# VKoskiv/c-ray

Measured on AMD Instinct MI355X. Metric: Mray/s (primary+secondary), higher is better.
Workload: dtype f32; 1 GPU; input/hdr.json 1280x720, 256 spp, 8 bounces (BASELINE.json configs[1]); venusscaled.obj = generated 524288-triangle stand-in (tools/gen_assets.py), HDR env map + 2048^2 grid texture from the reference tree; environment map: a generated stand-in of the HDR's size (tools/cfg2_blob.py — no reference tree to flatten hdr.json from): the same paths and rays, other radiance; parallelism=1 rank: the whole frame in one dispatch

## Files before the change

### c-ray_amd/csrc/cray_hip.hip

```cpp
#include <hip/hip_runtime.h>
#include <dlfcn.h>

#include <algorithm>
#include <chrono>
#include <cmath>
#include <cstdio>
#include <cstring>
#include <condition_variable>
#include <atomic>
#include <cassert>
#include <memory>
#include <mutex>
#include <thread>
#include <string>
#include <vector>

#include "cray_hip.h"
#define CRH_EM_POW_TABLES_IN_LDS
#include "pt_device.h"
#include "scene_compile.h"
#include "ctx_access.h"

using namespace crh;

// ... 929 lines not shown
	UP(prog, cs.prog.data(), cs.prog.size());
	UP(textures, cs.textures.data(), cs.textures.size());
	{
		void *texDev = nullptr;
		rc = takeTexels ? takeTexels(&texDev) : CRH_OK;
		if (rc) { freeScene(c); return rc; }
		if (texDev) { c->sceneAllocs.push_back(texDev); d.texels = (const f4 *)texDev; }
		else UP(texels, cs.texels.data(), cs.texels.size());
	}
#undef UP
	d.tlas_first = cs.tlas_first;
	d.material_count = (uint32_t)cs.materials.size(); d.bsdf_count = (uint32_t)cs.bsdfs.size(); d.const_count = (uint32_t)cs.consts.size();
	d.image_count = (uint32_t)cs.images.size(); d.texture_count = (uint32_t)cs.textures.size();
	d.tlas_root = cs.tlas_root; d.tlas_node_count = cs.tlas_node_count; d.tlas_prim_base = cs.tlas_prim_base; d.shade_classes = cs.shade_classes; d.instance_count = (uint32_t)cs.instances.size();
	d.background = cs.background;
	{ const crh_camera *cam = nullptr; rc = upload(c, &cs.camera, 1, &cam); if (rc) { freeScene(c); return rc; } d.camera = cam; }
	c->d = d;
	c->haveWide = !cs.wide.empty(); c->wideTlasRoot = cs.wide_tlas_root;
	if (cs.want_wide && !c->haveWide && !cs.wide_refused.empty())
		fprintf(stderr, "libcray_hip: CRH_WALK_WIDE4 was asked for, but this scene has no 4-ary copy (%s): the binary walk renders it\n", cs.wide_refused.c_str());
	c->hasPrograms = cs.prog.size() > 1 || cs.has_volumes || getenv("CRH_FORCE_PROGRAMS") != nullptr;
	c->hasVolumes = cs.has_volumes;
	c->aovDepth = cs.max_albedo_depth;
	c->haveScene = true;
	*tCopiesMs = upMs();
	rc = preloadKernel(c, true);
	if (rc != CRH_OK) return rc;
	unsigned int flag = 0;
	HIP_TRY(hipMemcpy(&flag, c->dWork + (CRH_WORK_SLOTS - 1), sizeof(flag), hipMemcpyDeviceToHost));
	return CRH_OK;
}
// ... 1428 lines not shown
```

### c-ray_amd/csrc/pathtrace_roll.h

```cpp
#pragma once

#define CRH_ROLL_HITS_MAX 136u
#define CRH_ROLL_IDS_MISSES (CRH_IDS_HITS + 2u * CRH_ROLL_HITS_MAX)
#define CRH_ROLL_IDS_BYTES (CRH_ROLL_IDS_MISSES + 128u)
#ifndef CRH_ROLL_SLOTS
#define CRH_ROLL_SLOTS 4u
#endif
#ifndef CRH_ROLL_FIFO
#define CRH_ROLL_FIFO 0
#endif
#define CRH_ROLL_SLOT_SHIFT 30u
#define CRH_ROLL_ITEM_MASK 0x3FFFFFFFu


template <int LEVEL, int WPS, bool PROG, int SAMP, bool WIDE = false>
__global__ __launch_bounds__(CRH_BLOCK, CRH_WPS_OVERRIDE) void k_pathtrace_roll(const DScene Sarg, const crh_render_params P, const BlockQueue Q, float *fb,
																 unsigned long long *counters,
																 float *stage, int chunk, unsigned long long *waveStats, const Sched K, float *queues, uint32_t *ovfAll, unsigned int *errFlag) {
	__shared__ uint32_t s_stack[CRH_STACK_LDS * CRH_BLOCK];
	__shared__ uint32_t s_park[CRH_PARK_SLOTS * CRH_BLOCK];
	enum { RQ_RAYS, RQ_HITS, RQ_MISSES, RQ_FREE, RQ_CLS_LO, RQ_CLS_HI,
	       RQ_GENLEFT,
	       RQ_FLAGS,
	       RQ_HEAD,
	       RQ_OPEN,
	       RQ_GEN,
	       RQ_DRY,
	       RQ_SLOT0 };
	enum { SJ_X0, SJ_Y0, SJ_WH , SJ_BWBH , SJ_PASS0, SJ_PASSN, SJ_NEXT, SJ_OUT,
	       SJ_BASE_LO, SJ_BASE_HI,
	       SJ_WORDS };
	enum { SJ_WH_DEFER = 1 << 30 };
	enum { SJ_WH_H_MASK = 0x3FFF };
#define CRH_RQ_IS_DRY(v) ((v) != 0)
	enum { NS = (int)CRH_ROLL_SLOTS, RQ_WORDS = RQ_SLOT0 + NS * SJ_WORDS };
	static_assert(NS >= 2 && NS <= 4, "2..4 job slots (two bits of the item word)");
	static_assert((CRH_STACK_LDS + CRH_PARK_SLOTS) * CRH_BLOCK * 4 + (CRH_BLOCK / 64) * (CRH_ROLL_IDS_BYTES + RQ_WORDS * 4) + 512 + 256 + CRH_INST_LDS_BYTES + CRH_SHADE_LDS_BYTES <= 40960, "4 blocks per CU share 160 KB of LDS (incl. powf's tables)");
	const DScene S = globalize(Sarg);
	CRH_EM_POW_TABLES_INIT();
	const unsigned long long tStart = wall_clock64();
	uint32_t unitsDone = 0;
#ifdef CRH_EXP_ABS_TIMES
	unsigned long long tDry = 0;
	bool snapDone = false;
#endif
	LdsStack stk;
	stk.lds = (lds_u32 *)&s_stack[threadIdx.x];
	stk.parkp = (lds_u32 *)&s_park[threadIdx.x];
	CRH_STAGE_SHADE_TABLES();
	CRH_STAGE_INSTANCE_TABLES();
	CountersT<LEVEL, PROG, WIDE> cnt;
	memset(&cnt, 0, sizeof(cnt));
	const uint32_t lane = threadIdx.x & 63u;
	const uint32_t wave = (blockIdx.x * CRH_BLOCK + threadIdx.x) >> 6;
	__shared__ uint8_t s_cls[256];
	const bool sorted = K.sortFrom > 0 && S.shade_classes >= (uint32_t)K.sortFrom && S.instance_count <= 256u;
	if (sorted) {
		for (uint32_t i = threadIdx.x; i < S.instance_count; i += CRH_BLOCK) s_cls[i] = (uint8_t)CRH_DINST_CLASS(S.instances[i].kind);
		__syncthreads();
	}
	stk.ovf = (glb_u32 *)ovfAll + (size_t)__builtin_amdgcn_readfirstlane(wave) * CRH_OVF_WORDS_PER_WAVE;
	const size_t slabFloats = (size_t)Q.bw * Q.bh * chunk * 3;
	float *const myStage = stage + (size_t)__builtin_amdgcn_readfirstlane(wave) * (size_t)NS * slabFloats;
	const int passEnd = P.first_pass + P.pass_count;
	const uint32_t trisOff = (uint32_t)((const char *)S.tris - (const char *)S.nodes);
	constexpr bool LEANTAB = CRH_PATH_LEAN && !PROG;
// ... 36 lines not shown
		if (open > 0) {
			lds_int *gj = wq + RQ_SLOT0 + wq[RQ_GEN] * SJ_WORDS, *oj = wq + RQ_SLOT0 + head * SJ_WORDS;
			const int gb = gj[SJ_BWBH], ob = oj[SJ_BWBH];
			left = (gb & 0xFFFF) * (gb >> 16) * gj[SJ_PASSN] - gj[SJ_NEXT];
			if (left < 0) left = 0;
			moreChunks = !(gj[SJ_WH] & SJ_WH_DEFER) && gj[SJ_PASS0] + gj[SJ_PASSN] < passEnd;
			if (oj[SJ_NEXT] >= (ob & 0xFFFF) * (ob >> 16) * oj[SJ_PASSN] && oj[SJ_OUT] == 0 && (open > 1 || !moreChunks)) flags |= 1;
		}
		if (open < NS && (!CRH_RQ_IS_DRY(wq[RQ_DRY]) || moreChunks)) flags |= 2;
		wq[RQ_GENLEFT] = left; wq[RQ_FLAGS] = flags;
	};

	if (lane == 0) {
		wq[RQ_RAYS] = 0; wq[RQ_HITS] = 0; wq[RQ_MISSES] = 0; wq[RQ_FREE] = (int)CRH_PATHS; wq[RQ_CLS_LO] = 0; wq[RQ_CLS_HI] = 0;
		wq[RQ_HEAD] = 0; wq[RQ_OPEN] = 0; wq[RQ_GEN] = 0; wq[RQ_DRY] = 0;
		for (int i = 0; i < NS * SJ_WORDS; ++i) wq[RQ_SLOT0 + i] = 0;
		refreshJobWords();
	}
	for (uint32_t i = lane; i < CRH_PATHS; i += 64u) ids[i] = (uint8_t)i;
	__threadfence_block();
	Walk w;
	memset(&w, 0, sizeof(w));
	w.phase = PH_IDLE;
	uint32_t myPath = 0;
	auto retireRefill = [&](int &rq, int &hq, int &mq) __attribute__((always_inline)) {
		const bool fin = (w.phase == PH_SHADE);
		const bool finHit = fin && w.hit.inst >= 0, finMiss = fin && w.hit.inst < 0;
		const unsigned long long hm = __ballot(finHit), mm = __ballot(finMiss);
		uint32_t cls = 0;
		if (fin) {
// ... 34 lines not shown
		if (idle && (int)er < take) {
			myPath = myRay;
#else
		if (idle && (int)er < take) {
			myPath = ids[CRH_IDS_RAYS + (uint32_t)(rq - take) + er];
#endif
			const f4 *q = tab.rec(myPath);
			const f4 q0 = q[0], q1 = q[1];
			{ TablePort<SAMP> port2{tab.rec(myPath)}; walkBegin(S, w, stk, v3{q0.x, q0.y, q0.z}, v3{q1.x, q1.y, q1.z}, cnt, port2, (uint32_t)K.rayFlags); }
			if constexpr (LEVEL >= 2) {
				if (dumpRays && dumpCount + er < dumpCap) { float *o = dumpRays + (size_t)(dumpCount + er) * 6u; o[0] = q0.x; o[1] = q0.y; o[2] = q0.z; o[3] = q1.x; o[4] = q1.y; o[5] = q1.z; }
			}
		}
		if constexpr (LEVEL >= 2) dumpCount += (uint32_t)take;
		hq += (int)__popcll(hm); mq += (int)__popcll(mm); rq -= take;
		if (lane == 0) { wq[RQ_HITS] = hq; wq[RQ_MISSES] = mq; wq[RQ_RAYS] = rq; }
		__threadfence_block();
	};
	uint32_t guard = (uint32_t)K.roundLimit;
	for (;;) {
		if (--guard == 0u) { if (lane == 0) atomicOr(errFlag, CRH_ERRFLAG_ROUND_LIMIT); break; }
#ifdef CRH_EXP_ABS_TIMES
		if (waveStats && !snapDone && (guard & 15u) == 0u) {
			uint32_t handedOut = 0;
			if (lane == 0) handedOut = __hip_atomic_load((uint32_t *)Q.counter, __ATOMIC_RELAXED, __HIP_MEMORY_SCOPE_AGENT);
			handedOut = __builtin_amdgcn_readfirstlane(handedOut);
			if (handedOut >= Q.total) {
				snapDone = true;
				if (lane == 0) {
					const int head = wq[RQ_HEAD], open = wq[RQ_OPEN];
					unsigned long long notGenerated = 0, notStaged = 0;
// ... 59 lines not shown
					const bool isT = nTw >= K.triInRun && w.phase == PH_TRI;
					if constexpr (LEVEL >= 2) {
						if (lane == 0) { CRH_WCTR(11, 1); CRH_WCTR(17, now); }
#ifdef CRH_CENSUS
						const uint32_t wf = (uint32_t)__popcll(__ballot(w.phase == PH_SHADE || w.phase == PH_IDLE));
						if (lane == 0) { CRH_WCTR(30, nTw >= K.triInRun ? 0u : (uint32_t)nTw); CRH_WCTR(31, wf); if (nTw >= K.triInRun) { CRH_WCTR(26, 1); CRH_WCTR(27, nTw); } }
#endif
					}
					if (isN || isT) {
						const uint32_t off = isN ? (uint32_t)(w.node << (WIDE ? 4 : 5)) : trisOff + w.pA * 48u;
						const char *rec = (const char *)S.nodes + off;
						q0 = *(const f4 *)rec; q1 = *(const f4 *)(rec + 16); q2 = *(const f4 *)(rec + 32); q3 = *(const f4 *)(rec + 48);
						if (WIDE || isT) { q4 = *(const f4 *)(rec + 64); q5 = *(const f4 *)(rec + 80); }
						if (WIDE && isN) { q6 = *(const f4 *)(rec + 96); q7 = *(const f4 *)(rec + 112); }
					}
					if constexpr (WIDE) { if (isN) stepWideLoaded<true>(S, w, stk, cnt, port, q0, q1, q2, q3, q4, q5, q6, q7); }
					else
					if (isN) stepNodeLoaded<true>(S, w, stk, cnt, port, q0, q1, q2, q3);
					if (isT) stepTriLoaded(S, w, stk, cnt, port, q0, q1, q2, q3, q4, q5);
					if ((int)__popcll(__ballot(w.phase == PH_CTRL)) >= K.ctrlInRun) {
#ifdef CRH_CENSUS
						if constexpr (LEVEL >= 2) { const uint32_t n2 = (uint32_t)__popcll(__ballot(w.phase == PH_CTRL)); if (lane == 0) { CRH_WCTR(28, 1); CRH_WCTR(29, n2); } }
#endif
						if (w.phase == PH_CTRL) stepCtrl(S, w, stk, cnt, port);
					}
					{
						const int nFi = (int)__popcll(__ballot(w.phase == PH_SHADE)), nEi = (int)__popcll(__ballot(w.phase == PH_IDLE));
						if (nFi + nEi >= K.swapInRun && (nFi > 0 || rqRun > 0) && hqRun < 64 && mqRun < 64) {
							if constexpr (LEVEL >= 2) { if (lane == 0) { CRH_WCTR(21, 1); CRH_WCTR(23, nFi + min(nEi + nFi, rqRun)); } }
							retireRefill(rqRun, hqRun, mqRun);
							port = TablePort<SAMP>{tab.rec(myPath)};
						}
					}
					now = __popcll(__ballot(w.phase == PH_NODE));
// ... 87 lines not shown
				const BlockJob J = loadJob(g);
				const uint32_t genNext = (uint32_t)wq[RQ_SLOT0 + g * SJ_WORDS + SJ_NEXT], genItems = genNext + (uint32_t)itemsLeft;
				const uint32_t item = genNext + lane;
				int x = 0, y = 0, pass = 0;
				const bool valid = item < genItems && decodeItem(J, item, x, y, pass);
				const unsigned long long vm = __ballot(valid);
				const int n = (int)__popcll(vm);
				if constexpr (COOP_STORE) {
					f4 q0 = f4{0.0f, 0.0f, 0.0f, 0.0f}, q1 = q0, q2 = q0, q3 = q0;
					uint32_t id = 0;
					if (valid) {
						const uint32_t rk = laneRank(vm);
						id = ids[CRH_IDS_FREE_END - (uint32_t)freeQ + rk];
						v3 ro, rd;
						PathRecT<RngT<SAMP>> r;
						beginPath(S, P, x, y, pass, ro, rd, r, cnt);
						packPathRay(q0, q1, q2, q3, ro, rd, r, item | ((uint32_t)g << CRH_ROLL_SLOT_SHIFT));
						ids[CRH_IDS_RAYS + (uint32_t)raysQ + rk] = (uint8_t)id;
					}
					tab.storeRec4(id, valid, q0, q1, q2, q3);
				} else
				if (valid) {
					const uint32_t rk = laneRank(vm);
					const uint32_t id = ids[CRH_IDS_FREE_END - (uint32_t)freeQ + rk];
					v3 ro, rd;
					PathRecT<RngT<SAMP>> r;
					beginPath(S, P, x, y, pass, ro, rd, r, cnt);
					putPathRay(tab.rec(id), ro, rd, r, item | ((uint32_t)g << CRH_ROLL_SLOT_SHIFT));
					ids[CRH_IDS_RAYS + (uint32_t)raysQ + rk] = (uint8_t)id;
				}
				if (lane == 0) {
					wq[RQ_RAYS] = raysQ + n; wq[RQ_FREE] = freeQ - n;
					lds_int *j = wq + RQ_SLOT0 + g * SJ_WORDS;
					j[SJ_NEXT] = (int)(genNext + 64u); j[SJ_OUT] = j[SJ_OUT] + n;
					refreshJobWords();
				}
				__threadfence_block();
				break;
			}
			case ST_MISS: {
				const int n = min(missQn, 64);
				int mySlot = -1;
				const bool have = (int)lane < n;
				uint32_t id = 0;
				f4 q0, q1, q2, q3;
				if constexpr (COOP_LOAD_MISS) {
					if (have) id = ids[CRH_ROLL_IDS_MISSES + (uint32_t)(missQn - n) + lane];
					tab.loadRec4(id, have, q0, q1, q2, q3);
				}
// ... 163 lines not shown
	}
	if (waveStats && lane == 0) {
#ifdef CRH_EXP_ABS_TIMES
		const unsigned long long tEnd = wall_clock64();
		waveStats[2 * wave] = tStart;
		waveStats[2 * wave + 1] = (((tDry ? tDry : tEnd) - tStart) << 32) | ((tEnd - tStart) & 0xFFFFFFFFull);
		if (!snapDone) { const size_t waves = (size_t)gridDim.x * (CRH_BLOCK / 64u); waveStats[2 * (waves + wave)] = 0; waveStats[2 * (waves + wave) + 1] = 0; }
#else
		waveStats[2 * wave] = wall_clock64() - tStart;
		waveStats[2 * wave + 1] = unitsDone;
#endif
	}
	const bool lead = (lane == 0);
	if constexpr (LEVEL >= 2) { if (dumpRays && lead) waveStats[CRH_DUMP_HDR + 2 + wave] = min(dumpCount, dumpCap); }
	uint32_t v;
	v = waveSum(cnt.paths); if (lead && v) atomicAdd(&counters[0], (unsigned long long)v);
	v = waveSum(cnt.rays); if (lead && v) atomicAdd(&counters[1], (unsigned long long)v);
	if constexpr (LEVEL >= 2) {
		v = waveSum(cnt.node_tests); if (lead && v) atomicAdd(&counters[2], (unsigned long long)v);
		v = waveSum(cnt.tri_tests); if (lead && v) atomicAdd(&counters[3], (unsigned long long)v);
		v = waveSum(cnt.inst_visits); if (lead && v) atomicAdd(&counters[4], (unsigned long long)v);
		v = waveSum(cnt.inst_hits); if (lead && v) atomicAdd(&counters[5], (unsigned long long)v);
		v = waveSum(cnt.sphere_tests); if (lead && v) atomicAdd(&counters[6], (unsigned long long)v);
		v = waveSum(cnt.tex_fetches); if (lead && v) atomicAdd(&counters[7], (unsigned long long)v);
	}
}
#undef CRH_WCTR
```

### c-ray_amd/csrc/pt_device.h

```cpp
#pragma once
#include <stdint.h>
#include <math.h>
#include <float.h>
#include <type_traits>
#include <utility>
#include "cray_hip.h"
#include "exact_math.h"

#if defined(__HIPCC__)
#define CRH_DEV __device__ __forceinline__
#define CRH_DEV_NOINLINE __device__ __noinline__
#define CRH_MEM __device__ __forceinline__
#else
#define CRH_MEM inline __attribute__((always_inline))
#define CRH_DEV static inline __attribute__((always_inline))
#define CRH_DEV_NOINLINE static __attribute__((noinline))
#endif

namespace crh {

#define CRH_PI 3.141592653589793238462643383279502f
#define CRH_NONE 0xFFFFFFFFu

struct alignas(16) f4 { float x, y, z, w; };
// ... 97 lines not shown
	uint32_t t_setup, t_trav, t_shade;
	uint32_t w_node, w_tri, w_ctrl, w_round, w_shade, w_setup;
	uint32_t u_node, u_shade;
	uint32_t t_swap, t_gen, n_swap, n_gen, u_swap, u_tri, u_ctrl;
#ifdef CRH_CENSUS
	uint32_t w_tri_in, u_tri_in, w_ctrl_in, u_ctrl_in;
	uint32_t u_wait_tri, u_wait_fin;
#endif
};
template <bool PROGRAMS, bool WIDE> struct CountersT<1, PROGRAMS, WIDE> {
	static constexpr int level = 1;
	static constexpr bool programs = PROGRAMS;
	static constexpr bool wide = WIDE;
	uint32_t rays, paths;
};
typedef CountersT<2, true> Counters;
typedef CountersT<1, true> LiteCounters;
struct NoCounters { static constexpr int level = 0; static constexpr bool programs = true; static constexpr bool wide = false; };
template <class T> struct cnt_traits { static constexpr int level = T::level; static constexpr bool programs = T::programs; static constexpr bool wide = T::wide; };
template <class T> struct cnt_traits<T &> { static constexpr int level = T::level; static constexpr bool programs = T::programs; static constexpr bool wide = T::wide; };
#define CRH_COUNT(c, field, n) do { if constexpr (crh::cnt_traits<decltype(c)>::level >= 2) (c).field += (n); } while (0)
#if defined(__HIPCC__)
#define CRH_TICK() ((uint32_t)wall_clock64())
#else
#define CRH_TICK() 0u
#endif
#define CRH_COUNT1(c, field, n) do { if constexpr (crh::cnt_traits<decltype(c)>::level >= 1) (c).field += (n); } while (0)

CRH_DEV v3 vadd(v3 a, v3 b) { return v3{a.x + b.x, a.y + b.y, a.z + b.z}; }
CRH_DEV v3 vsub(v3 a, v3 b) { return v3{a.x - b.x, a.y - b.y, a.z - b.z}; }
// ... 226 lines not shown
			  (m.c.x * v.x) + (m.c.y * v.y) + (m.c.z * v.z)};
}
CRH_DEV v3 xfVectorT(v3 v, const InstLine &m) {
	return v3{(m.a.x * v.x) + (m.b.x * v.y) + (m.c.x * v.z),
			  (m.a.y * v.x) + (m.b.y * v.y) + (m.c.y * v.z),
			  (m.a.z * v.x) + (m.b.z * v.y) + (m.c.z * v.z)};
}

CRH_DEV float triangleDistribution(float v) {
	const float orig = v * 2.0f - 1.0f;
	v = orig / sqrtf(fabsf(orig));
	v = rmin(rmax(v, -1.0f), 1.0f);
	v = v - ((orig >= 0.0f) ? 1.0f : -1.0f);
	return v;
}
template <class R>
CRH_DEV void getCameraRay(const crh_camera &cam, R &rng, int x, int y, v3 &ro, v3 &rd) {
	const v3 right = v3{cam.right[0], cam.right[1], cam.right[2]};
	const v3 up = v3{cam.up[0], cam.up[1], cam.up[2]};
	const v3 forward = v3{cam.forward[0], cam.forward[1], cam.forward[2]};
	v3 start = v3{0.0f, 0.0f, 0.0f};
	const float jitterX = triangleDistribution(getDimension(rng));
	const float jitterY = triangleDistribution(getDimension(rng));
	v3 pixX = vscale(right, (cam.sensor[0] / (float)cam.width));
	v3 pixY = vscale(up, (cam.sensor[1] / (float)cam.height));
	v3 pixV = vadd(forward, vadd(vscale(pixX, (float)x - (float)cam.width * 0.5f + jitterX + 0.5f),
								 vscale(pixY, (float)y - (float)cam.height * 0.5f + jitterY + 0.5f)));
	v3 dir = vnorm(pixV);
	if (cam.aperture > 0.0f) {
		float ft = cam.focal_distance / vdot(dir, forward);
		v3 focusPoint = alongRay(start, dir, ft);
		v2 disc = randomCoordOnUnitDisc(rng);
		v2 lensPoint = v2{disc.x * cam.aperture, disc.y * cam.aperture};
		start = vadd(start, vadd(vscale(right, lensPoint.x), vscale(up, lensPoint.y)));
		dir = vnorm(vsub(focusPoint, start));
	}
	ro = xfPoint(start, cam.A);
	rd = xfVector(dir, cam.A);
}

CRH_DEV uint32_t wrapIndex(int i, uint32_t W, uint32_t m64) {
	if ((W & (W - 1u)) == 0u) return (uint32_t)i & (W - 1u);
// ... 378 lines not shown
	RayK k;
	uint32_t node;
	uint32_t pA, pAe, pB, pBe;
	uint32_t sp, spBase;
	uint32_t inBlas, instFound;
	int32_t curInst;
	TravHit hit;
};

struct NullPort {
	CRH_MEM float draw() { return 0.5f; }
	CRH_MEM void save(int, uint32_t) {}
	CRH_MEM uint32_t load(int) { return 0u; }
};
enum { VP_T, VP_U, VP_V, VP_SLOT, VP_T1, VP_WORDS };
enum { BLAS_NONE = 0, BLAS_SOLID = 1, BLAS_VOL_ENTRY = 2, BLAS_VOL_EXIT = 3 };

template <class Cnt>
CRH_DEV bool sphereTest(const v3 o, const v3 d, float radius, float bound, float &t, Cnt &cnt) {
	CRH_COUNT(cnt, sphere_tests, 1);
	const float A = vdot(d, d);
	const float B = 2.0f * vdot(d, o);
	const float C = vdot(o, o) - (radius * radius);
	const float disc = B * B - 4.0f * A * C;
	if (disc < 0.0f) return false;
	const float sq = sqrtf(disc);
	float t0 = (-B + sq) / 2.0f;
	const float t1 = (-B - sq) / 2.0f;
	if (t0 > t1 && t1 > 0.0f) t0 = t1;
	if (t0 < 0.00001f || t0 > bound) return false;
	t = t0;
// ... 31 lines not shown
		return false;
	}
	if (w.inBlas == BLAS_VOL_EXIT && found) {
		float t1 = asF32(port.load(VP_T1));
		if (t1 < 0.0f) t1 = 0.0f;
		const float distanceInsideVolume = tWalk;
		const float hitDistance = -(1.0f / instDensity(instLine(S, stk, w.curInst, 1))) * em::logf_(port.draw());
		if (hitDistance < distanceInsideVolume) {
			w.hit.t = t1 + hitDistance; w.hit.u = 0.0f; w.hit.v = 0.0f; w.hit.slot = -2; w.hit.inst = w.curInst;
			CRH_COUNT(cnt, inst_hits, 1);
		}
	}
	return false;
}

template <class Stack, class Cnt, class Port>
CRH_DEV void walkAdvance(const DScene &S, Walk &w, Stack &stk, Cnt &cnt, Port &port) {
	if (w.pA != w.pAe) { w.phase = w.inBlas ? PH_TRI : PH_CTRL; return; }
	if constexpr (cnt_traits<Cnt>::wide) {
		if (w.node == CRH_NONE && w.sp > w.spBase) {
			const uint32_t e = stk.pop(--w.sp);
			if (e & CRH_WREF_LEAF) { w.pA = e & CRH_WREF_FIRST_MASK; w.pAe = w.pA + ((e >> CRH_WREF_COUNT_SHIFT) & CRH_WREF_COUNT_MAX); w.phase = w.inBlas ? PH_TRI : PH_CTRL; return; }
			w.node = e;
		}
	} else {
		if (w.node == CRH_NONE && w.sp > w.spBase) w.node = stk.pop(--w.sp);
	}
	if (w.node != CRH_NONE) { w.phase = w.k.oct >> CRH_RAY_PHASE_SHIFT; return; }
	if (!w.inBlas) { w.phase = PH_SHADE; return; }
	if constexpr (cnt_traits<Cnt>::programs) {
		if (__builtin_expect(w.inBlas >= BLAS_VOL_ENTRY, 0)) { if (volumeAdvance(S, w, stk, cnt, port)) return; }
	}
	if (w.instFound) { w.hit.inst = w.curInst; CRH_COUNT(cnt, inst_hits, 1); }
// ... 91 lines not shown
	walkAdvance(S, w, stk, cnt, port);
}
template <bool FAST = true, class Stack, class Cnt, class Port>
CRH_DEV void stepWide(const DScene &S, Walk &w, Stack &stk, Cnt &cnt, Port &port) {
	const char *rec = (const char *)S.nodes + (uint32_t)(w.node << 4);
	const f4 a0 = *(const f4 *)rec, a1 = *(const f4 *)(rec + 16), b0 = *(const f4 *)(rec + 32), b1 = *(const f4 *)(rec + 48);
	const f4 c0 = *(const f4 *)(rec + 64), c1 = *(const f4 *)(rec + 80), d0 = *(const f4 *)(rec + 96), d1 = *(const f4 *)(rec + 112);
	stepWideLoaded<FAST>(S, w, stk, cnt, port, a0, a1, b0, b1, c0, c1, d0, d1);
}
template <bool FAST, class Stack, class Cnt, class Port>
CRH_DEV void stepNodeAny(const DScene &S, Walk &w, Stack &stk, Cnt &cnt, Port &port) {
	if constexpr (cnt_traits<Cnt>::wide) stepWide<FAST>(S, w, stk, cnt, port); else stepNode<FAST>(S, w, stk, cnt, port);
}

template <class Cnt>
CRH_DEV void testTriangle(const f4 q0, const f4 q1, const f4 q2, uint32_t slot, Walk &w, Cnt &cnt) {
	const v3 v0 = v3{q0.x, q0.y, q0.z}, e1 = v3{q0.w, q1.x, q1.y}, e2 = v3{q1.z, q1.w, q2.x}, n = v3{q2.y, q2.z, q2.w};
	CRH_COUNT(cnt, tri_tests, 1);
	const v3 c = vsub(v0, w.k.o);
	const v3 r = vcross(w.k.d, c);
	const float invDet = 1.0f / vdot(n, w.k.d);
	const float u = vdot(r, e2) * invDet;
	const float v = vdot(r, e1) * invDet;
	if (u >= 0.0f && v >= 0.0f && u + v <= 1.0f) {
		const float t = vdot(n, c) * invDet;
		if (t >= 0.0f && t < w.hit.t) { w.hit.t = t; w.hit.u = u; w.hit.v = v; w.hit.slot = (int32_t)slot; w.instFound = 1; }
	}
}
template <class Stack, class Cnt, class Port>
CRH_DEV void stepTriLoaded(const DScene &S, Walk &w, Stack &stk, Cnt &cnt, Port &port, const f4 a0, const f4 a1, const f4 a2, const f4 b0, const f4 b1, const f4 b2) {
	const uint32_t slot = w.pA;
	const bool two = slot + 1u < w.pAe;
	const uint32_t slot2 = two ? slot + 1u : slot;
	w.pA = slot2 + 1u;
	if (w.pA == w.pAe) { w.pA = w.pB; w.pAe = w.pBe; w.pB = w.pBe = 0; }
	testTriangle(a0, a1, a2, slot, w, cnt);
	if (two) testTriangle(b0, b1, b2, slot2, w, cnt);
	walkAdvance(S, w, stk, cnt, port);
}
template <class Stack, class Cnt, class Port>
CRH_DEV void stepTri(const DScene &S, Walk &w, Stack &stk, Cnt &cnt, Port &port) {
	const uint32_t slot = w.pA;
	const uint32_t slot2 = slot + 1u < w.pAe ? slot + 1u : slot;
	const char *ta = (const char *)S.tris + (uint32_t)(slot * 48u), *tb = (const char *)S.tris + (uint32_t)(slot2 * 48u);
	const f4 a0 = *(const f4 *)ta, a1 = *(const f4 *)(ta + 16), a2 = *(const f4 *)(ta + 32);
	const f4 b0 = *(const f4 *)tb, b1 = *(const f4 *)(tb + 16), b2 = *(const f4 *)(tb + 32);
	stepTriLoaded(S, w, stk, cnt, port, a0, a1, a2, b0, b1, b2);
}

template <class Stack, class Cnt, class Port>
CRH_DEV void stepCtrl(const DScene &S, Walk &w, Stack &stk, Cnt &cnt, Port &port) {
	const uint32_t slot = w.pA++;
	if (w.pA == w.pAe) { w.pA = w.pB; w.pAe = w.pBe; w.pB = w.pBe = 0; }
	const int32_t idx = (int32_t)(slot - S.tlas_prim_base);
	const InstLine inst = instLine(S, stk, idx, 0);
	CRH_COUNT(cnt, inst_visits, 1);
	v3 o = xfPoint(w.k.o, inst);
	const v3 d = xfVector(w.k.d, inst);
	o = vadd(o, vscale(d, instRayOffset(inst)));
	const uint32_t kind = CRH_DINST_KIND(instKind(inst));
	const bool volume = cnt_traits<Cnt>::programs && (instKind(inst) & CRH_DINST_VOLUME) != 0u;
	if (kind == CRH_DINST_SPHERE) {
		float t0;
		if (__builtin_expect(volume, 0)) {
			float tExit;
			if (sphereTest(o, d, instRadius(inst), w.hit.t, t0, cnt) && sphereTest(alongRay(o, d, t0 + 0.0001f), d, instRadius(inst), w.hit.t, tExit, cnt)) {
				if (t0 < 0.0f) t0 = 0.0f;
				const float hitDistance = -(1.0f / instDensity(instLine(S, stk, idx, 1))) * em::logf_(port.draw());
				if (hitDistance < tExit) {
					w.hit.t = t0 + hitDistance; w.hit.u = 0.0f; w.hit.v = 0.0f; w.hit.slot = -2; w.hit.inst = idx;
					CRH_COUNT(cnt, inst_hits, 1);
				}
			}
		} else if (sphereTest(o, d, instRadius(inst), w.hit.t, t0, cnt)) {
			w.hit.t = t0; w.hit.slot = -1; w.hit.inst = idx;
			CRH_COUNT(cnt, inst_hits, 1);
// ... 1 lines not shown
	} else if (kind == CRH_DINST_MESH_EMPTY) {
		if (!volume) w.hit.inst = -1;
	} else if (!(w.k.oct & CRH_RAY_LITERAL) && (o.x != o.x || o.y != o.y || o.z != o.z || d.x != d.x || d.y != d.y || d.z != d.z)) {
	} else {
		RayK ko = makeRayK(o, d);
		ko.oct |= w.k.oct & CRH_RAY_LITERAL;
		bool enter = true;
		uint32_t rootA = 0, rootAe = 0;
		if (kind == CRH_DINST_MESH_LEAF) {
			const f4 n0 = S.nodes[2u * instRoot(inst)], n1 = S.nodes[2u * instRoot(inst) + 1u];
			float tE;
			CRH_COUNT(cnt, node_tests, 1);
			enter = intersectNode(n0, n1, ko, w.hit.t, tE);
			rootA = CRH_DNODE_FIRST(n1); rootAe = rootA + CRH_DNODE_COUNT(n1);
		}
		if (enter) {
			if (!sceneIsOneInstance(S)) {
			stk.park(PK_NODE, w.node); stk.park(PK_PA, w.pA); stk.park(PK_PAE, w.pAe); stk.park(PK_PB, w.pB); stk.park(PK_PBE, w.pBe);
			stk.park(PK_OX, asU32(w.k.o.x)); stk.park(PK_OY, asU32(w.k.o.y)); stk.park(PK_OZ, asU32(w.k.o.z));
			stk.park(PK_DX, asU32(w.k.d.x)); stk.park(PK_DY, asU32(w.k.d.y)); stk.park(PK_DZ, asU32(w.k.d.z));
			stk.park(PK_IX, asU32(w.k.inv.x)); stk.park(PK_IY, asU32(w.k.inv.y)); stk.park(PK_IZ, asU32(w.k.inv.z));
			stk.park(PK_OCT, w.k.oct);
			}
			if (kind == CRH_DINST_MESH_LEAF) { w.node = CRH_NONE; w.pA = rootA; w.pAe = rootAe; }
			else { w.node = cnt_traits<Cnt>::wide ? asU32(instRadius(inst))  : instRoot(inst); w.pA = w.pAe = 0; }
			w.pB = w.pBe = 0;
			w.spBase = w.sp; w.inBlas = BLAS_SOLID; w.instFound = 0; w.curInst = idx; w.k = ko;
			if (__builtin_expect(volume, 0)) {
				w.inBlas = BLAS_VOL_ENTRY;
				port.save(VP_T, asU32(w.hit.t)); port.save(VP_U, asU32(w.hit.u)); port.save(VP_V, asU32(w.hit.v)); port.save(VP_SLOT, (uint32_t)w.hit.slot);
// ... 101 lines not shown

template <class R> struct PathRecT { float wr, wg, wb; float fr, fg, fb; R rng; int depth; };
typedef PathRecT<Rng> PathRec;

CRH_DEV bool decodeItem(const BlockJob &J, uint32_t item, int &x, int &y, int &pass) {
	const uint32_t pc = (uint32_t)J.passCount, bw = (uint32_t)J.bw;
	const bool pcPow2 = (pc & (pc - 1u)) == 0u;
	const uint32_t pcShift = 31u - (uint32_t)__builtin_clz(pc | 1u), bwShift = 31u - (uint32_t)__builtin_clz(bw | 1u);
	const uint32_t pix = pcPow2 ? (item >> pcShift) : (item / pc);
	const int px = (int)(pix & (bw - 1u)), py = (int)(pix >> bwShift);
	x = J.x0 + px; y = J.y0 + py;
	pass = J.passBegin + (int)(pcPow2 ? (item & (pc - 1u)) : (item - pix * pc));
	return px < J.w && py < J.h;
}

template <class PR, class Cnt>
CRH_DEV void beginPath(const DScene &S, const crh_render_params &P, int x, int y, int pass, v3 &ro, v3 &rd, PR &r, Cnt &cnt) {
	CRH_COUNT1(cnt, paths, 1);
	const uint32_t pixIdx = (uint32_t)(y * P.image_width + x);
	initSampler(r.rng, pass, P.max_passes, pixIdx);
	getCameraRay(*S.camera, r.rng, x, y, ro, rd);
	r.wr = r.wg = r.wb = 1.0f; r.fr = r.fg = r.fb = 0.0f; r.depth = 0;
}

template <class PR, class Cnt, class Src = GlobalTables>
CRH_DEV bool shadeCore(const DScene &S, const crh_render_params &P, v3 &ro, v3 &rd, const TravHit &hit, PR &r, Cnt &cnt, const Src &src = Src()) {
	ShadeRec rec;
	rec.dir = rd;
	if (hit.inst < 0) {
		rec.point = v3{0.0f, 0.0f, 0.0f}; rec.normal = v3{0.0f, 0.0f, 0.0f}; rec.uv = v2{0.0f, 0.0f};
		rec.distance = hit.t; rec.ior = 0.0f;
		const rgba bg = sampleBackground(S, rec, cnt, src);
		r.fr = r.fr + (r.wr * bg.r); r.fg = r.fg + (r.wg * bg.g); r.fb = r.fb + (r.wb * bg.b);
		return false;
	}
	const HitInfo h = finishHit<true, cnt_traits<Cnt>::programs>(S, ro, rd, hit, src);
// ... 102 lines not shown
```

### c-ray_amd/csrc/scene_compile.cpp

```cpp
#include "scene_compile.h"

#include <algorithm>
#include <cstdio>
#include <cstdlib>
#include <cstring>
#include <chrono>
#include <map>
#include <mutex>
#include <thread>

namespace crh {

namespace {

struct Fail {
	int code;
	std::string msg;
};

#define CHECK(cond, code, ...)                                 \
	do {                                                       \
		if (!(cond)) {                                         \
			char buf_[256];                                    \
			snprintf(buf_, sizeof(buf_), __VA_ARGS__);         \
// ... 339 lines not shown
			out.bsdfs[g] = d;
		}
		if (out.consts.empty()) addConst(0, 0, 0, 0);
		if (out.images.empty()) out.images.push_back(DImage{CRH_NONE, 0});
		if (out.prog.empty()) { DOp end; memset(&end, 0, sizeof(end)); end.kind = CRH_OP_END; out.prog.push_back(end); }
	}

	void run() {
		auto t0 = std::chrono::steady_clock::now();
		auto lap = [&]() { const auto t1 = std::chrono::steady_clock::now(); const double ms = std::chrono::duration<double, std::milli>(t1 - t0).count(); t0 = t1; return ms; };
		CHECK(s->struct_size == sizeof(crh_scene_desc), CRH_ERR_INVALID, "crh_scene_desc.struct_size %u != %zu", s->struct_size, sizeof(crh_scene_desc));
		CHECK(s->abi_version == CRH_SCENE_VERSION, CRH_ERR_INVALID, "scene description version %u != %d", s->abi_version, CRH_SCENE_VERSION);
		CHECK(s->node_count < 0x3FFFFFFFull && s->prim_index_count < 0x3FFFFFFFull && s->poly_count < 0x7FFFFFFFull, CRH_ERR_UNSUPPORTED, "scene too large for 32-bit device indices");
		CHECK(s->camera.width > 0 && s->camera.height > 0, CRH_ERR_INVALID, "camera has no image size");
		out.camera = s->camera;

		{
			uint64_t texelTotal = 0, nodeTotal = 4;
			for (uint64_t t = 0; t < s->texture_count; ++t) texelTotal += (uint64_t)s->textures[t].width * s->textures[t].height;
			for (uint64_t m = 0; m < s->mesh_count; ++m) nodeTotal += ((uint64_t)s->meshes[m].node_count + 3) * 2;
			nodeTotal += ((uint64_t)s->tlas_node_count + 3) * 2;
			if (texelTotal < 0xFFFFFFFFull) out.texels.reserve((size_t)std::max<uint64_t>(texelTotal, 1));
			if (nodeTotal < 0xFFFFFFFFull) out.nodes.reserve((size_t)nodeTotal);
		}
		for (uint64_t t = 0; t < s->texture_count; ++t) {
			const crh_texture &tx = s->textures[t];
			CHECK(tx.width > 0 && tx.height > 0 && (tx.channels == 1 || tx.channels == 3 || tx.channels == 4), CRH_ERR_INVALID, "texture %llu has a bad shape", (unsigned long long)t);
			const uint64_t bytes = (uint64_t)tx.width * tx.height * tx.channels * (tx.is_float ? 4u : 1u);
			CHECK(tx.offset % 4 == 0 && tx.offset + bytes <= s->texture_bytes, CRH_ERR_INVALID, "texture %llu data out of bounds", (unsigned long long)t);
			CHECK(!tx.has_alpha || tx.channels == 4, CRH_ERR_INVALID, "texture %llu: has_alpha needs 4 channels", (unsigned long long)t);
// ... 293 lines not shown
```

### c-ray_amd/csrc/scene_compile.h

```cpp
#pragma once
#include <cstdlib>
#include <cstring>
#include <sys/mman.h>
#include <functional>
#include <new>
#include <string>
#include <vector>
#include "pt_device.h"

namespace crh {

#define CRH_PODBUF_HUGE_PAGE ((size_t)2 << 20)
#define CRH_PODBUF_HUGE_FROM ((size_t)8 << 20)
template <class T> struct PodBuf {
	T *p = nullptr;
	size_t n = 0, cap = 0;
	PodBuf() = default;
	PodBuf(const PodBuf &) = delete;
	PodBuf &operator=(const PodBuf &) = delete;
	~PodBuf() { free(p); }
	T *data() { return p; }
	const T *data() const { return p; }
	size_t size() const { return n; }
	bool empty() const { return n == 0; }
// ... 36 lines not shown
	std::vector<DOp> prog;
	std::vector<DTexture> textures;
	PodBuf<f4> texels;
	uint32_t tlas_root = 0, tlas_node_count = 0, tlas_prim_base = 0, background = 0, shade_classes = 0;
	uint32_t tlas_first = 0;
	uint32_t max_stack = 0;
	uint32_t max_add_depth = 0;
	uint32_t max_albedo_depth = 0;
	PodBuf<f4> wide;
	uint32_t wide_tlas_root = 0;
	uint32_t wide_max_stack = 0;
	bool want_wide = false;
	std::string wide_refused;
	bool has_volumes = false;
	crh_camera camera;
};

inline size_t sceneNodeBytes(const CompiledScene &c) { return (c.nodes.size() * sizeof(f4) + 255u) & ~(size_t)255u; }
inline size_t sceneWideOffset(const CompiledScene &c) { return (sceneNodeBytes(c) + c.tris.size() * sizeof(f4) + 96u + 127u) & ~(size_t)127u; }

int compile_scene(const crh_scene_desc *scene, CompiledScene &out, std::string &err, const std::function<void()> &texelsReady = std::function<void()>());

}
```

Baseline: 9168 Mray/s.

## Hoist camera pixel terms, add leaf-instance walk and wave-level counters

Camera pixel-step vectors and half-size terms are now computed once on the host and stored after the camera record, so primary ray generation skips two divides and scales per path. This hoist is enabled by default. Two more paths sit behind compile flags that default off: counting rays and paths per wave in LDS instead of per lane, and a lighter walk for single-leaf mesh instances that parks the instance-space ray. Visit-census instrumentation is added as well. The default change only affects primary ray setup, which is a small share of the work, and it depends on the camera record layout cast being correct.

```diff
diff --git a/c-ray_amd/csrc/cray_hip.hip b/c-ray_amd/csrc/cray_hip.hip
--- a/c-ray_amd/csrc/cray_hip.hip
+++ b/c-ray_amd/csrc/cray_hip.hip
@@ -967,7 +967,7 @@
 	d.image_count = (uint32_t)cs.images.size(); d.texture_count = (uint32_t)cs.textures.size();
 	d.tlas_root = cs.tlas_root; d.tlas_node_count = cs.tlas_node_count; d.tlas_prim_base = cs.tlas_prim_base; d.shade_classes = cs.shade_classes; d.instance_count = (uint32_t)cs.instances.size();
 	d.background = cs.background;
-	{ const crh_camera *cam = nullptr; rc = upload(c, &cs.camera, 1, &cam); if (rc) { freeScene(c); return rc; } d.camera = cam; }
+	{ const DCameraRec rec{cs.camera, cs.camera_terms}; const DCameraRec *cam = nullptr; rc = upload(c, &rec, 1, &cam); if (rc) { freeScene(c); return rc; } d.camera = &cam->cam; }
 	c->d = d;
 	c->haveWide = !cs.wide.empty(); c->wideTlasRoot = cs.wide_tlas_root;
 	if (cs.want_wide && !c->haveWide && !cs.wide_refused.empty())
diff --git a/c-ray_amd/csrc/pathtrace_roll.h b/c-ray_amd/csrc/pathtrace_roll.h
--- a/c-ray_amd/csrc/pathtrace_roll.h
+++ b/c-ray_amd/csrc/pathtrace_roll.h
@@ -26,7 +26,9 @@
 	       RQ_OPEN,
 	       RQ_GEN,
 	       RQ_DRY,
-	       RQ_SLOT0 };
+	       RQ_FIXED };
+	constexpr bool WAVE_COUNT = CRH_WAVE_COUNT1 && LEVEL == 1;
+	enum { RQ_NRAYS = RQ_FIXED, RQ_NPATHS = RQ_FIXED + 1, RQ_SLOT0 = RQ_FIXED + (WAVE_COUNT ? 2 : 0) };
 	enum { SJ_X0, SJ_Y0, SJ_WH , SJ_BWBH , SJ_PASS0, SJ_PASSN, SJ_NEXT, SJ_OUT,
 	       SJ_BASE_LO, SJ_BASE_HI,
 	       SJ_WORDS };
@@ -49,7 +51,7 @@
 	stk.parkp = (lds_u32 *)&s_park[threadIdx.x];
 	CRH_STAGE_SHADE_TABLES();
 	CRH_STAGE_INSTANCE_TABLES();
-	CountersT<LEVEL, PROG, WIDE> cnt;
+	typename std::conditional<WAVE_COUNT, WaveCountedT<PROG, WIDE>, CountersT<LEVEL, PROG, WIDE>>::type cnt;
 	memset(&cnt, 0, sizeof(cnt));
 	const uint32_t lane = threadIdx.x & 63u;
 	const uint32_t wave = (blockIdx.x * CRH_BLOCK + threadIdx.x) >> 6;
@@ -116,6 +118,7 @@
 	if (lane == 0) {
 		wq[RQ_RAYS] = 0; wq[RQ_HITS] = 0; wq[RQ_MISSES] = 0; wq[RQ_FREE] = (int)CRH_PATHS; wq[RQ_CLS_LO] = 0; wq[RQ_CLS_HI] = 0;
 		wq[RQ_HEAD] = 0; wq[RQ_OPEN] = 0; wq[RQ_GEN] = 0; wq[RQ_DRY] = 0;
+		if constexpr (WAVE_COUNT) { wq[RQ_NRAYS] = 0; wq[RQ_NPATHS] = 0; }
 		for (int i = 0; i < NS * SJ_WORDS; ++i) wq[RQ_SLOT0 + i] = 0;
 		refreshJobWords();
 	}
@@ -180,7 +183,10 @@
 		}
 		if constexpr (LEVEL >= 2) dumpCount += (uint32_t)take;
 		hq += (int)__popcll(hm); mq += (int)__popcll(mm); rq -= take;
-		if (lane == 0) { wq[RQ_HITS] = hq; wq[RQ_MISSES] = mq; wq[RQ_RAYS] = rq; }
+		if (lane == 0) {
+			wq[RQ_HITS] = hq; wq[RQ_MISSES] = mq; wq[RQ_RAYS] = rq;
+			if constexpr (WAVE_COUNT) { if (take > 0) wq[RQ_NRAYS] = wq[RQ_NRAYS] + take; }
+		}
 		__threadfence_block();
 	};
 	uint32_t guard = (uint32_t)K.roundLimit;
@@ -270,10 +276,19 @@
 						if (WIDE || isT) { q4 = *(const f4 *)(rec + 64); q5 = *(const f4 *)(rec + 80); }
 						if (WIDE && isN) { q6 = *(const f4 *)(rec + 96); q7 = *(const f4 *)(rec + 112); }
 					}
+#ifdef CRH_CENSUS_VISITS
+					const uint32_t inBefore = w.inBlas;
+#endif
 					if constexpr (WIDE) { if (isN) stepWideLoaded<true>(S, w, stk, cnt, port, q0, q1, q2, q3, q4, q5, q6, q7); }
 					else
 					if (isN) stepNodeLoaded<true>(S, w, stk, cnt, port, q0, q1, q2, q3);
 					if (isT) stepTriLoaded(S, w, stk, cnt, port, q0, q1, q2, q3, q4, q5);
+#ifdef CRH_CENSUS_VISITS
+					{
+						const uint32_t nl = (uint32_t)__popcll(__ballot(inBefore != 0u && w.inBlas == 0u)), ng = (uint32_t)__popcll(__ballot(inBefore != 0u && inBefore != BLAS_LEAF && w.inBlas == 0u));
+						if (lane == 0) { CRH_VISIT_CENSUS(VC_NODE_ITERS, 1); if (nl) { CRH_VISIT_CENSUS(VC_LEAVE_ITERS, 1); CRH_VISIT_CENSUS(VC_LEAVE_LANES, nl); } if (ng) { CRH_VISIT_CENSUS(VC_LEAVE_GEN_ITERS, 1); CRH_VISIT_CENSUS(VC_LEAVE_GEN_LANES, ng); } }
+					}
+#endif
 					if ((int)__popcll(__ballot(w.phase == PH_CTRL)) >= K.ctrlInRun) {
 #ifdef CRH_CENSUS
 						if constexpr (LEVEL >= 2) { const uint32_t n2 = (uint32_t)__popcll(__ballot(w.phase == PH_CTRL)); if (lane == 0) { CRH_WCTR(28, 1); CRH_WCTR(29, n2); } }
@@ -391,7 +406,7 @@
 						id = ids[CRH_IDS_FREE_END - (uint32_t)freeQ + rk];
 						v3 ro, rd;
 						PathRecT<RngT<SAMP>> r;
-						beginPath(S, P, x, y, pass, ro, rd, r, cnt);
+						beginPath<CRH_GEN_HOIST != 0>(S, P, x, y, pass, ro, rd, r, cnt);
 						packPathRay(q0, q1, q2, q3, ro, rd, r, item | ((uint32_t)g << CRH_ROLL_SLOT_SHIFT));
 						ids[CRH_IDS_RAYS + (uint32_t)raysQ + rk] = (uint8_t)id;
 					}
@@ -402,7 +417,7 @@
 					const uint32_t id = ids[CRH_IDS_FREE_END - (uint32_t)freeQ + rk];
 					v3 ro, rd;
 					PathRecT<RngT<SAMP>> r;
-					beginPath(S, P, x, y, pass, ro, rd, r, cnt);
+					beginPath<CRH_GEN_HOIST != 0>(S, P, x, y, pass, ro, rd, r, cnt);
 					putPathRay(tab.rec(id), ro, rd, r, item | ((uint32_t)g << CRH_ROLL_SLOT_SHIFT));
 					ids[CRH_IDS_RAYS + (uint32_t)raysQ + rk] = (uint8_t)id;
 				}
@@ -410,6 +425,7 @@
 					wq[RQ_RAYS] = raysQ + n; wq[RQ_FREE] = freeQ - n;
 					lds_int *j = wq + RQ_SLOT0 + g * SJ_WORDS;
 					j[SJ_NEXT] = (int)(genNext + 64u); j[SJ_OUT] = j[SJ_OUT] + n;
+					if constexpr (WAVE_COUNT) wq[RQ_NPATHS] = wq[RQ_NPATHS] + n;
 					refreshJobWords();
 				}
 				__threadfence_block();
@@ -603,8 +619,15 @@
 	const bool lead = (lane == 0);
 	if constexpr (LEVEL >= 2) { if (dumpRays && lead) waveStats[CRH_DUMP_HDR + 2 + wave] = min(dumpCount, dumpCap); }
 	uint32_t v;
+	if constexpr (WAVE_COUNT) {
+		if (lead) {
+			v = (uint32_t)wq[RQ_NPATHS]; if (v) atomicAdd(&counters[0], (unsigned long long)v);
+			v = (uint32_t)wq[RQ_NRAYS]; if (v) atomicAdd(&counters[1], (unsigned long long)v);
+		}
+	} else {
 	v = waveSum(cnt.paths); if (lead && v) atomicAdd(&counters[0], (unsigned long long)v);
 	v = waveSum(cnt.rays); if (lead && v) atomicAdd(&counters[1], (unsigned long long)v);
+	}
 	if constexpr (LEVEL >= 2) {
 		v = waveSum(cnt.node_tests); if (lead && v) atomicAdd(&counters[2], (unsigned long long)v);
 		v = waveSum(cnt.tri_tests); if (lead && v) atomicAdd(&counters[3], (unsigned long long)v);
diff --git a/c-ray_amd/csrc/pt_device.h b/c-ray_amd/csrc/pt_device.h
--- a/c-ray_amd/csrc/pt_device.h
+++ b/c-ray_amd/csrc/pt_device.h
@@ -135,6 +135,35 @@
 	static constexpr bool wide = WIDE;
 	uint32_t rays, paths;
 };
+#ifndef CRH_WAVE_COUNT1
+#define CRH_WAVE_COUNT1 0
+#endif
+#ifndef CRH_GEN_HOIST
+#define CRH_GEN_HOIST 1
+#endif
+#ifndef CRH_LEAF_VISIT
+#define CRH_LEAF_VISIT 0
+#endif
+#if defined(CRH_CENSUS_VISITS) && !defined(__HIPCC__)
+}
+#include <cstdio>
+namespace crh {
+enum { VC_SPHERE, VC_LEAF, VC_LEAF_IN, VC_MESH, VC_LEAVE_ITERS, VC_LEAVE_LANES, VC_LEAVE_GEN_ITERS, VC_LEAVE_GEN_LANES, VC_NODE_ITERS, VC_COUNT };
+inline unsigned long long g_visitCensus[VC_COUNT];
+struct VisitCensusPrinter {
+	~VisitCensusPrinter() {
+		static const char *const names[VC_COUNT] = {"sphere_visits", "leaf_mesh_visits", "leaf_mesh_entered", "mesh_visits", "leave_iters", "leave_lanes", "general_leave_iters", "general_leave_lanes", "node_iters"};
+		fprintf(stderr, "VISIT_CENSUS");
+		for (int i = 0; i < VC_COUNT; ++i) fprintf(stderr, " %s=%llu", names[i], g_visitCensus[i]);
+		fprintf(stderr, "\n");
+	}
+};
+inline VisitCensusPrinter g_visitCensusPrinter;
+#define CRH_VISIT_CENSUS(k, n) __atomic_fetch_add(&crh::g_visitCensus[crh::k], (unsigned long long)(n), __ATOMIC_RELAXED)
+#else
+#define CRH_VISIT_CENSUS(k, n) do {} while (0)
+#endif
+template <bool PROGRAMS, bool WIDE> struct WaveCountedT { static constexpr int level = 0; static constexpr bool programs = PROGRAMS; static constexpr bool wide = WIDE; };
 typedef CountersT<2, true> Counters;
 typedef CountersT<1, true> LiteCounters;
 struct NoCounters { static constexpr int level = 0; static constexpr bool programs = true; static constexpr bool wide = false; };
@@ -391,7 +420,16 @@
 	v = v - ((orig >= 0.0f) ? 1.0f : -1.0f);
 	return v;
 }
-template <class R>
+struct CameraTerms { float pixX[3], pixY[3]; float halfW, halfH; };
+struct DCameraRec { crh_camera cam; CameraTerms terms; };
+inline CameraTerms cameraTerms(const crh_camera &cam) {
+	CameraTerms t;
+	const float sx = cam.sensor[0] / (float)cam.width, sy = cam.sensor[1] / (float)cam.height;
+	for (int i = 0; i < 3; ++i) { t.pixX[i] = cam.right[i] * sx; t.pixY[i] = cam.up[i] * sy; }
+	t.halfW = (float)cam.width * 0.5f; t.halfH = (float)cam.height * 0.5f;
+	return t;
+}
+template <bool HOIST = false, class R>
 CRH_DEV void getCameraRay(const crh_camera &cam, R &rng, int x, int y, v3 &ro, v3 &rd) {
 	const v3 right = v3{cam.right[0], cam.right[1], cam.right[2]};
 	const v3 up = v3{cam.up[0], cam.up[1], cam.up[2]};
@@ -399,10 +437,18 @@
 	v3 start = v3{0.0f, 0.0f, 0.0f};
 	const float jitterX = triangleDistribution(getDimension(rng));
 	const float jitterY = triangleDistribution(getDimension(rng));
-	v3 pixX = vscale(right, (cam.sensor[0] / (float)cam.width));
-	v3 pixY = vscale(up, (cam.sensor[1] / (float)cam.height));
-	v3 pixV = vadd(forward, vadd(vscale(pixX, (float)x - (float)cam.width * 0.5f + jitterX + 0.5f),
-								 vscale(pixY, (float)y - (float)cam.height * 0.5f + jitterY + 0.5f)));
+	v3 pixV;
+	if constexpr (HOIST) {
+		const CameraTerms &t = ((const DCameraRec *)&cam)->terms;
+		const v3 pixX = v3{t.pixX[0], t.pixX[1], t.pixX[2]}, pixY = v3{t.pixY[0], t.pixY[1], t.pixY[2]};
+		pixV = vadd(forward, vadd(vscale(pixX, (float)x - t.halfW + jitterX + 0.5f),
+								  vscale(pixY, (float)y - t.halfH + jitterY + 0.5f)));
+	} else {
+		v3 pixX = vscale(right, (cam.sensor[0] / (float)cam.width));
+		v3 pixY = vscale(up, (cam.sensor[1] / (float)cam.height));
+		pixV = vadd(forward, vadd(vscale(pixX, (float)x - (float)cam.width * 0.5f + jitterX + 0.5f),
+								  vscale(pixY, (float)y - (float)cam.height * 0.5f + jitterY + 0.5f)));
+	}
 	v3 dir = vnorm(pixV);
 	if (cam.aperture > 0.0f) {
 		float ft = cam.focal_distance / vdot(dir, forward);
@@ -811,7 +857,8 @@
 	CRH_MEM uint32_t load(int) { return 0u; }
 };
 enum { VP_T, VP_U, VP_V, VP_SLOT, VP_T1, VP_WORDS };
-enum { BLAS_NONE = 0, BLAS_SOLID = 1, BLAS_VOL_ENTRY = 2, BLAS_VOL_EXIT = 3 };
+enum { BLAS_NONE = 0, BLAS_SOLID = 1, BLAS_VOL_ENTRY = 2, BLAS_VOL_EXIT = 3,
+       BLAS_LEAF = 4 };
 
 template <class Cnt>
 CRH_DEV bool sphereTest(const v3 o, const v3 d, float radius, float bound, float &t, Cnt &cnt) {
@@ -873,9 +920,17 @@
 	return false;
 }
 
-template <class Stack, class Cnt, class Port>
+template <bool MAYLEAF = false, class Stack, class Cnt, class Port>
 CRH_DEV void walkAdvance(const DScene &S, Walk &w, Stack &stk, Cnt &cnt, Port &port) {
 	if (w.pA != w.pAe) { w.phase = w.inBlas ? PH_TRI : PH_CTRL; return; }
+	if constexpr (MAYLEAF && CRH_LEAF_VISIT && !cnt_traits<Cnt>::wide) {
+		if (w.inBlas == BLAS_LEAF) {
+			if (w.instFound) { w.hit.inst = w.curInst; CRH_COUNT(cnt, inst_hits, 1); }
+			w.inBlas = 0; w.instFound = 0;
+			w.pA = stk.unpark(PK_PA); w.pAe = stk.unpark(PK_PAE); w.pB = stk.unpark(PK_PB); w.pBe = stk.unpark(PK_PBE);
+			if (w.pA != w.pAe) { w.phase = PH_CTRL; return; }
+		}
+	}
 	if constexpr (cnt_traits<Cnt>::wide) {
 		if (w.node == CRH_NONE && w.sp > w.spBase) {
 			const uint32_t e = stk.pop(--w.sp);
@@ -997,12 +1052,21 @@
 }
 
 template <class Cnt>
+#if CRH_LEAF_VISIT
+CRH_DEV void testTriangle(const f4 q0, const f4 q1, const f4 q2, uint32_t slot, Walk &w, const v3 o, const v3 d, Cnt &cnt) {
+	const v3 v0 = v3{q0.x, q0.y, q0.z}, e1 = v3{q0.w, q1.x, q1.y}, e2 = v3{q1.z, q1.w, q2.x}, n = v3{q2.y, q2.z, q2.w};
+	CRH_COUNT(cnt, tri_tests, 1);
+	const v3 c = vsub(v0, o);
+	const v3 r = vcross(d, c);
+	const float invDet = 1.0f / vdot(n, d);
+#else
 CRH_DEV void testTriangle(const f4 q0, const f4 q1, const f4 q2, uint32_t slot, Walk &w, Cnt &cnt) {
 	const v3 v0 = v3{q0.x, q0.y, q0.z}, e1 = v3{q0.w, q1.x, q1.y}, e2 = v3{q1.z, q1.w, q2.x}, n = v3{q2.y, q2.z, q2.w};
 	CRH_COUNT(cnt, tri_tests, 1);
 	const v3 c = vsub(v0, w.k.o);
 	const v3 r = vcross(w.k.d, c);
 	const float invDet = 1.0f / vdot(n, w.k.d);
+#endif
 	const float u = vdot(r, e2) * invDet;
 	const float v = vdot(r, e1) * invDet;
 	if (u >= 0.0f && v >= 0.0f && u + v <= 1.0f) {
@@ -1017,9 +1081,22 @@
 	const uint32_t slot2 = two ? slot + 1u : slot;
 	w.pA = slot2 + 1u;
 	if (w.pA == w.pAe) { w.pA = w.pB; w.pAe = w.pBe; w.pB = w.pBe = 0; }
+#if CRH_LEAF_VISIT
+	v3 o = w.k.o, d = w.k.d;
+	if constexpr (!cnt_traits<Cnt>::wide) {
+		if (w.inBlas == BLAS_LEAF) {
+			o = v3{asF32(stk.unpark(PK_OX)), asF32(stk.unpark(PK_OY)), asF32(stk.unpark(PK_OZ))};
+			d = v3{asF32(stk.unpark(PK_DX)), asF32(stk.unpark(PK_DY)), asF32(stk.unpark(PK_DZ))};
+		}
+	}
+	testTriangle(a0, a1, a2, slot, w, o, d, cnt);
+	if (two) testTriangle(b0, b1, b2, slot2, w, o, d, cnt);
+	walkAdvance<true>(S, w, stk, cnt, port);
+#else
 	testTriangle(a0, a1, a2, slot, w, cnt);
 	if (two) testTriangle(b0, b1, b2, slot2, w, cnt);
 	walkAdvance(S, w, stk, cnt, port);
+#endif
 }
 template <class Stack, class Cnt, class Port>
 CRH_DEV void stepTri(const DScene &S, Walk &w, Stack &stk, Cnt &cnt, Port &port) {
@@ -1043,6 +1120,7 @@
 	o = vadd(o, vscale(d, instRayOffset(inst)));
 	const uint32_t kind = CRH_DINST_KIND(instKind(inst));
 	const bool volume = cnt_traits<Cnt>::programs && (instKind(inst) & CRH_DINST_VOLUME) != 0u;
+	CRH_VISIT_CENSUS(VC_SPHERE + (kind == CRH_DINST_SPHERE ? 0 : kind == CRH_DINST_MESH_LEAF ? 1 : 3), 1);
 	if (kind == CRH_DINST_SPHERE) {
 		float t0;
 		if (__builtin_expect(volume, 0)) {
@@ -1074,6 +1152,14 @@
 			enter = intersectNode(n0, n1, ko, w.hit.t, tE);
 			rootA = CRH_DNODE_FIRST(n1); rootAe = rootA + CRH_DNODE_COUNT(n1);
 		}
+		if (enter && kind == CRH_DINST_MESH_LEAF) CRH_VISIT_CENSUS(VC_LEAF_IN, 1);
+		if (CRH_LEAF_VISIT && !cnt_traits<Cnt>::wide && enter && kind == CRH_DINST_MESH_LEAF && !volume && rootA != rootAe && !sceneIsOneInstance(S) && !(w.k.oct & CRH_RAY_LITERAL)) {
+			stk.park(PK_PA, w.pA); stk.park(PK_PAE, w.pAe); stk.park(PK_PB, w.pB); stk.park(PK_PBE, w.pBe);
+			stk.park(PK_OX, asU32(o.x)); stk.park(PK_OY, asU32(o.y)); stk.park(PK_OZ, asU32(o.z));
+			stk.park(PK_DX, asU32(d.x)); stk.park(PK_DY, asU32(d.y)); stk.park(PK_DZ, asU32(d.z));
+			w.pA = rootA; w.pAe = rootAe; w.pB = w.pBe = 0;
+			w.inBlas = BLAS_LEAF; w.instFound = 0; w.curInst = idx;
+		} else
 		if (enter) {
 			if (!sceneIsOneInstance(S)) {
 			stk.park(PK_NODE, w.node); stk.park(PK_PA, w.pA); stk.park(PK_PAE, w.pAe); stk.park(PK_PB, w.pB); stk.park(PK_PBE, w.pBe);
@@ -1205,12 +1291,12 @@
 	return px < J.w && py < J.h;
 }
 
-template <class PR, class Cnt>
+template <bool HOIST = false, class PR, class Cnt>
 CRH_DEV void beginPath(const DScene &S, const crh_render_params &P, int x, int y, int pass, v3 &ro, v3 &rd, PR &r, Cnt &cnt) {
 	CRH_COUNT1(cnt, paths, 1);
 	const uint32_t pixIdx = (uint32_t)(y * P.image_width + x);
 	initSampler(r.rng, pass, P.max_passes, pixIdx);
-	getCameraRay(*S.camera, r.rng, x, y, ro, rd);
+	getCameraRay<HOIST>(*S.camera, r.rng, x, y, ro, rd);
 	r.wr = r.wg = r.wb = 1.0f; r.fr = r.fg = r.fb = 0.0f; r.depth = 0;
 }
 
diff --git a/c-ray_amd/csrc/scene_compile.cpp b/c-ray_amd/csrc/scene_compile.cpp
--- a/c-ray_amd/csrc/scene_compile.cpp
+++ b/c-ray_amd/csrc/scene_compile.cpp
@@ -377,6 +377,7 @@
 		CHECK(s->node_count < 0x3FFFFFFFull && s->prim_index_count < 0x3FFFFFFFull && s->poly_count < 0x7FFFFFFFull, CRH_ERR_UNSUPPORTED, "scene too large for 32-bit device indices");
 		CHECK(s->camera.width > 0 && s->camera.height > 0, CRH_ERR_INVALID, "camera has no image size");
 		out.camera = s->camera;
+		out.camera_terms = cameraTerms(out.camera);
 
 		{
 			uint64_t texelTotal = 0, nodeTotal = 4;
diff --git a/c-ray_amd/csrc/scene_compile.h b/c-ray_amd/csrc/scene_compile.h
--- a/c-ray_amd/csrc/scene_compile.h
+++ b/c-ray_amd/csrc/scene_compile.h
@@ -74,6 +74,7 @@
 	std::string wide_refused;
 	bool has_volumes = false;
 	crh_camera camera;
+	CameraTerms camera_terms;
 };
 
 inline size_t sceneNodeBytes(const CompiledScene &c) { return (c.nodes.size() * sizeof(f4) + 255u) & ~(size_t)255u; }
```

After: 9190 Mray/s, median of 6. About the same (+0.2%).
